# NikNazarov/TorchPIV

Measured on AMD Instinct MI355X. Metric: image-pairs/sec at 4 MP, wind=64 ov=32 2-pass CWS; % HBM roofline, higher is better.
Workload: dtype u32 exact sums + f64 / f32

## Files before the change

### include/torchpiv_hip.h

```cpp
#ifndef TORCHPIV_HIP_H
#define TORCHPIV_HIP_H

#include <stddef.h>
#include <stdint.h>

#ifdef __cplusplus
extern "C" {
#endif

#define TPIV_VERSION 2

enum tpiv_status {
    TPIV_OK = 0,
    TPIV_EINVAL = 1,
    TPIV_EKEY = 2,
    TPIV_EHIP = 3,
    TPIV_ENOMEM = 4,
    TPIV_EUNSUPPORTED = 5
};

enum tpiv_mode {
    TPIV_MODE_DWS = 1,
    TPIV_MODE_CWS = 2,
    TPIV_MODE_CWS_FAST = 3
// ... 115 lines not shown

int tpiv_read_files(const char* const* paths, int n_files, uint8_t* dst, size_t slot_bytes, int n_threads,
                    int64_t* sizes);

typedef struct tpiv_reader tpiv_reader;
tpiv_reader* tpiv_reader_open(const char* const* paths, int64_t n_files, int files_per_batch, uint8_t* const* bufs,
                              int n_bufs, size_t slot_bytes, int n_threads);
int tpiv_reader_next(tpiv_reader* reader, int* n_files, int* buf_index, int64_t* sizes);
int tpiv_reader_release(tpiv_reader* reader);
void tpiv_reader_close(tpiv_reader* reader);


int tpiv_plan_set_timing(tpiv_plan* plan, int enable);
int tpiv_plan_get_timing(tpiv_plan* plan, double* avg_ms, int n_slots, int* n_runs);
int tpiv_plan_exact_fallbacks(tpiv_plan* plan, long long* n_windows);
int tpiv_plan_exact_timing(const tpiv_plan* plan, double* ms4);


int tpiv_debug_pass(int mode, int precision, const uint8_t* a_dev, const uint8_t* b_dev, int batch, int H, int W,
                    int ws, int ov, const double* u2_dev, const double* v2_dev, const double* zero_dev,
                    double* u_dev, double* v_dev, uint8_t* invalid_dev,
                    float* win_dev, float* corr_dev, void* work_dev, size_t work_bytes, void* stream);

int tpiv_debug_iter_compact(int mode, const uint8_t* a_dev, const uint8_t* b_dev, int batch, int H, int W,
                            int ws, int ov, const double* u_raw_dev, const double* v_raw_dev, const uint8_t* mask_dev,
                            double val_ratio, int val_win, int precision,
                            double* u_dev, double* v_dev, uint8_t* invalid_dev, double* du_dev, double* dv_dev,
                            void* work_dev, size_t work_bytes, void* stream);

int tpiv_debug_peaks(const float* maps_dev, int n_maps, int ws, int planar, double val_ratio, int val_win,
                     double* u_dev, double* v_dev, uint8_t* invalid_dev,
                     void* work_dev, size_t work_bytes, void* stream);
// ... 10 lines not shown
```

### torchpiv_amd/_lib.py

```python
from __future__ import annotations

import ctypes as C
import os

_HERE = os.path.dirname(os.path.abspath(__file__))
LIB_PATH = os.environ.get("TPIV_LIB") or os.path.join(_HERE, "libtorchpiv_hip.so")

OK, EINVAL, EKEY, EHIP, ENOMEM, EUNSUPPORTED = 0, 1, 2, 3, 4, 5
MODE_DWS, MODE_CWS, MODE_CWS_FAST = 1, 2, 3
MODES = {"DWS": MODE_DWS, "CWS": MODE_CWS}
ITER_MODES = dict(MODES, CWS_Fast=MODE_CWS_FAST)
PREC_FAST, PREC_REFERENCE, PREC_F64, PREC_EXACT = 0, 1, 2, 3
PRECISIONS = {"fast": PREC_FAST, "reference": PREC_REFERENCE, "f64": PREC_F64, "exact": PREC_EXACT}
PREFILTER_NONE, PREFILTER_MIN, PREFILTER_MEAN = 0, 1, 2
PREFILTERS = {None: PREFILTER_NONE, "min": PREFILTER_MIN, "mean": PREFILTER_MEAN}
ABI_VERSION = 2


class HipError(RuntimeError):
    pass


def _load():
    if not os.path.exists(LIB_PATH):
# ... 19 lines not shown
    "tpiv_coordinates": (C.c_int, [_int, _int, _int, _int, C.POINTER(C.c_double), C.POINTER(C.c_double)]),
    "tpiv_spline_matrix": (C.c_int, [_int, C.POINTER(C.c_double), _int, C.POINTER(C.c_double),
                                     C.POINTER(C.c_double)]),
    "tpiv_pass1": (C.c_int, [_u8p, _u8p, _int, _int, _int, _int, _int, _dbl, _int, _int, _f64p, _f64p, _u8p,
                             _vp, C.c_size_t, _vp]),
    "tpiv_work_bytes": (C.c_size_t, [_int, _int, _int, _int, _int]),
    "tpiv_predict": (C.c_int, [_int, _int, _int, _int, _int, _int, _f64p, _f64p, _f64p, _f64p, _u8p,
                               _f64p, _f64p, _f64p, _f64p, _f64p, _vp]),
    "tpiv_iter": (C.c_int, [_int, _u8p, _u8p, _int, _int, _int, _int, _int, _f64p, _f64p, _f64p, _f64p,
                            _dbl, _int, _int, _f64p, _f64p, _u8p, _f64p, _f64p, _vp, C.c_size_t, _vp]),
    "tpiv_plan_create": (C.c_int, [C.POINTER(C.c_void_p), _int, _int, _int, _int, _int, _int, _dbl, _dbl,
                                   _int, _int, _int]),
    "tpiv_plan_kernel_name": (C.c_char_p, [C.c_void_p, _int, C.c_char_p, _int]),
    "tpiv_plan_exact_fallbacks": (_int, [C.c_void_p, C.POINTER(C.c_longlong)]),
    "tpiv_plan_exact_timing": (_int, [C.c_void_p, C.POINTER(C.c_double)]),
    "tpiv_plan_destroy": (None, [C.c_void_p]),
    "tpiv_plan_n_pass": (C.c_int, [C.c_void_p]),
    "tpiv_plan_pass_geometry": (C.c_int, [C.c_void_p, _int, C.POINTER(C.c_int), C.POINTER(C.c_int),
                                          C.POINTER(C.c_int), C.POINTER(C.c_int)]),
    "tpiv_plan_run": (C.c_int, [C.c_void_p, _u8p, _u8p, _int, _f64p, _f64p, _u8p, _vp]),
    "tpiv_plan_pass_fields": (C.c_int, [C.c_void_p, _int, C.POINTER(C.c_void_p), C.POINTER(C.c_void_p),
                                        C.POINTER(C.c_void_p)]),
    "tpiv_median_test": (C.c_int, [_f64p, _f64p, _u8p, _int, _int, _int, _dbl, _dbl, _int, _u8p, _f64p, _f64p, _vp]),
    "tpiv_plan_set_outlier": (C.c_int, [C.c_void_p, _int, _dbl, _dbl, _int]),
    "tpiv_plan_pass_outliers": (C.c_int, [C.c_void_p, _int, C.POINTER(C.c_void_p)]),
    "tpiv_postval": (C.c_int, [_f64p, _f64p, _u8p, _int, _int, _int, _u8p, _vp, _vp]),
    "tpiv_postval_compact": (C.c_int, [_f64p, _f64p, _u8p, _vp, _int, _int, _int, _vp, _vp, _f64p, _vp, _vp]),
    "tpiv_finish_fields": (C.c_int, [_f64p, _f64p, _int, _int, _int, C.c_double, C.c_double, _f64p, _f64p, _vp]),
    "tpiv_ensemble_moments": (C.c_int, [_f64p, _f64p, _int, C.c_longlong, _f64p, _vp]),
    "tpiv_bmp_unpack": (C.c_int, [_u8p, _vp, _u8p, _int, _int, _int, _u8p, _vp]),
# ... 49 lines not shown
```

### torchpiv_amd/csrc/c_api.cpp

```cpp
#include "../../include/torchpiv_hip.h"

#include <hip/hip_runtime.h>

#include <fcntl.h>
#include <sys/stat.h>
#include <unistd.h>

#include <algorithm>
#include <atomic>
#include <condition_variable>
#include <mutex>
#include <cmath>
#include <cstdio>
#include <cstring>
#include <string>
#include <thread>
#include <vector>

#include "piv_kernels.h"

namespace {

thread_local std::string g_err;
#ifdef TPIV_STAMPS
// ... 173 lines not shown
struct tpiv_plan {
    int H = 0, W = 0, n_pass = 0, mode = 0, max_batch = 0, val_win = 3, device = 0, precision = 0;
    double val_ratio = 1.2;
    std::vector<PassGeo> geo;
    std::vector<double*> u, v;
    std::vector<uint8_t*> val;
    std::vector<double*> Ay, Ax;
    std::vector<double*> Wy32, Ax32;
    std::vector<int*> k0y32, k0x32;
    std::vector<int> KY, KX;
    double *u0 = nullptr, *v0 = nullptr, *T = nullptr;
    uint8_t* pmask = nullptr;
    float* peak_raw = nullptr;
    size_t peak_raw_bytes = 0;
    int last_batch = 0;
    unsigned* exact_count = nullptr;
    int outlier_kind = 0, outlier_min = 3;
    double outlier_threshold = 2.0, outlier_eps = 0.1;
    std::vector<uint8_t*> ostatus;
    double *raw_u = nullptr, *raw_v = nullptr;
    uint8_t* raw_val = nullptr;
    std::vector<void*> allocs;
    bool timing = false;
    std::vector<std::vector<hipEvent_t>> events;
    size_t runs_recorded = 0;

    ~tpiv_plan() {
        for (void* p : allocs) (void)hipFree(p);
        for (auto& r : events)
            for (hipEvent_t e : r) (void)hipEventDestroy(e);
// ... 198 lines not shown
    q.v_c = v_c;
    q.val_c = invalid_c;
    q.T = work;
    q.u0 = u0;
    q.v0 = v0;
    q.u2 = u2;
    q.v2 = v2;
    HIP_TRY(tpiv::launch_predict(q, (hipStream_t)stream));
    return TPIV_OK;
}

static int run_iter(int mode, int precision, const uint8_t* a, const uint8_t* b, int batch, int H, int W, int ws,
                    int ov, const double* u0, const double* v0, const double* u2, const double* v2,
                    double val_ratio, int val_win, double* u, double* v, uint8_t* invalid, double* du,
                    double* dv, float* dbg_win, float* dbg_corr, void* work, size_t work_bytes, void* stream,
                    const uint8_t* pmask = nullptr) {
    if (mode != TPIV_MODE_DWS && mode != TPIV_MODE_CWS && mode != TPIV_MODE_CWS_FAST)
        return fail(TPIV_EKEY, "unknown multipass mode");
    int rc = check_window(H, W, ws, ov, val_win);
    if (rc) return rc;
    if (mode == TPIV_MODE_CWS_FAST && ws < 2) return fail(TPIV_EINVAL, "window too small");
    if (mode != TPIV_MODE_CWS_FAST && !pmask && (!u2 || !v2)) return fail(TPIV_EINVAL, "tpiv_iter: u2 / v2 missing");
    if (!u0 || !v0) return fail(TPIV_EINVAL, "tpiv_iter: u0 / v0 missing");
    if (!valid_precision(precision)) return fail(TPIV_EINVAL, "precision must be TPIV_PREC_FAST, TPIV_PREC_REFERENCE, TPIV_PREC_F64 or TPIV_PREC_EXACT");
    if (batch <= 0) return TPIV_OK;
    tpiv::PassParams p{};
    p.A = a;
    p.B = b;
    p.batch = batch;
    p.H = H;
    p.W = W;
// ... 4 lines not shown
    p.u0 = u0;
    p.v0 = v0;
    p.u2 = u2;
    p.v2 = v2;
    p.pmask = pmask;
    p.u = u;
    p.v = v;
    p.val = invalid;
    p.du = du;
    p.dv = dv;
    p.val_ratio = val_ratio;
    p.val_win = val_win;
    p.dbg_win = dbg_win;
    p.dbg_corr = dbg_corr;
    p.stamps = g_stamps;
    rc = check_work(work, work_bytes,
                    tpiv::peak_raw_bytes(ws, batch, p.n_rows * p.n_cols, TPIV_PREC_FAST, mode == TPIV_MODE_CWS_FAST));
    if (rc) return rc;
    p.peak_raw = static_cast<float*>(work);
    int n_cu;
    rc = n_cu_of_current_device(&n_cu);
    if (rc) return rc;
    HIP_TRY(tpiv::launch_xcorr(p, mode, n_cu, (hipStream_t)stream));
    return TPIV_OK;
}

int tpiv_iter(int mode, const uint8_t* a, const uint8_t* b, int batch, int H, int W, int ws, int ov,
              const double* u0, const double* v0, const double* u2, const double* v2,
              double val_ratio, int val_win, int precision, double* u, double* v, uint8_t* invalid, double* du,
              double* dv, void* work, size_t work_bytes, void* stream) {
// ... 130 lines not shown
            if (t_dense > max_T) max_T = t_dense;
        }
    }
    if (rc == TPIV_OK) {
        size_t raw = 0;
        for (size_t i = 0; i < pl->geo.size(); ++i) {
            const PassGeo& g = pl->geo[i];
            const size_t b = tpiv::peak_raw_bytes(g.ws, max_batch, g.n_rows * g.n_cols,
                                                  i == 0 ? precision : (int)TPIV_PREC_FAST);
            if (b > raw) raw = b;
        }
        pl->peak_raw_bytes = raw;
        if (raw) rc = pl->alloc(&pl->peak_raw, raw / sizeof(float) + 64);
        if (rc == TPIV_OK && precision == TPIV_PREC_EXACT && tpiv::exact_refine_size(pl->geo[0].ws))
            rc = pl->alloc(&pl->exact_count, 4);
    }
    if (rc == TPIV_OK && n_pass > 1) {
        rc = pl->alloc(&pl->u0, max_fine * max_batch);
        if (!rc) rc = pl->alloc(&pl->v0, max_fine * max_batch);
        if (!rc) rc = pl->alloc(&pl->pmask, max_fine * max_batch);
        if (!rc) rc = pl->alloc(&pl->T, max_T * max_batch);
    }
    if (rc) {
        const std::string keep = g_err;
        delete pl;
        g_err = keep;
        return rc;
    }
    *out = pl;
    return TPIV_OK;
// ... 18 lines not shown
    buf[0] = 0;
    if (!plan || pass < 0 || pass >= plan->n_pass) return buf;
    const int mode = pass == 0 ? (int)tpiv::MODE_PASS1 : plan->mode;
    return tpiv::xcorr_kernel_name(plan->geo[pass].ws, mode, plan->precision, buf, len);
}

int tpiv_plan_exact_fallbacks(tpiv_plan* plan, long long* n_windows) {
    if (!plan || !n_windows) return fail(TPIV_EINVAL, "null argument");
    if (!plan->exact_count)
        return fail(TPIV_EINVAL, "not a TPIV_PREC_EXACT plan with an even first-pass window size from 8 to 128");
    if (plan->last_batch <= 0) return fail(TPIV_EINVAL, "the plan has not run yet");
    HIP_TRY(hipDeviceSynchronize());
    unsigned n = 0;
    HIP_TRY(hipMemcpy(&n, plan->exact_count, sizeof(n), hipMemcpyDeviceToHost));
    *n_windows = (long long)n;
    return TPIV_OK;
}

int tpiv_plan_pass_fields(const tpiv_plan* plan, int pass, double** u, double** v, uint8_t** invalid) {
    if (!plan || pass < 0 || pass >= plan->n_pass - 1)
        return fail(TPIV_EINVAL, "only the passes before the last keep their fields in the plan");
    if (u) *u = plan->u[pass];
    if (v) *v = plan->v[pass];
    if (invalid) *invalid = plan->val[pass];
    return TPIV_OK;
}

static int run_banded_predict(tpiv_plan* plan, int p, int batch, const double* u_c, const double* v_c,
                              const uint8_t* val_c, double* u0, double* v0, double* u2, double* v2,
                              hipStream_t st, uint8_t* mask_out = nullptr) {
// ... 161 lines not shown
            if (!rc && plan->exact_count) {
                const size_t off = tpiv::exact_fallback_count_offset(batch, g.n_rows * g.n_cols);
                HIP_TRY(hipMemcpyAsync(plan->exact_count, reinterpret_cast<const char*>(plan->peak_raw) + off,
                                       sizeof(unsigned), hipMemcpyDeviceToDevice, st));
            }
        } else {
            const PassGeo& c = plan->geo[p - 1];
            mark(2 * p - 1, 0);
            rc = run_banded_predict(plan, p, batch, plan->u[p - 1], plan->v[p - 1], plan->val[p - 1], plan->u0,
                                    plan->v0, nullptr, nullptr, st, plan->pmask);
            mark(2 * p - 1, 1);
            mark(2 * p, 0);
            if (!rc)
                rc = run_iter(plan->mode, plan->precision, a, b, batch, plan->H, plan->W, g.ws, g.ov, plan->u0, plan->v0,
                              nullptr, nullptr, plan->val_ratio, plan->val_win, pu, pv, pval, nullptr,
                              nullptr, nullptr, nullptr, plan->peak_raw, plan->peak_raw_bytes, stream, plan->pmask);
            mark(2 * p, 1);
        }
        if (rc) return rc;
        if (test) {
            rc = run_median_test(pu, pv, pval, batch, g.n_rows, g.n_cols, plan->outlier_threshold, plan->outlier_eps,
                                 plan->outlier_min, plan->ostatus[p], p < last ? fu : nullptr, p < last ? fv : nullptr, 1,
                                 p < last ? nullptr : fval, st);
            if (rc) return rc;
        }
    }
    if (plan->timing && plan->runs_recorded < 512) plan->runs_recorded++;
    return TPIV_OK;
}

int tpiv_postval(double* u, double* v, const uint8_t* invalid, int batch, int n_rows, int n_cols, uint8_t* cls,
                 int32_t* counts, void* stream) {
    if (batch < 0 || n_rows < 1 || n_cols < 1) return fail(TPIV_EINVAL, "tpiv_postval: empty grid");
    if ((long long)n_rows * n_cols >= (1LL << 31)) return fail(TPIV_EUNSUPPORTED, "field too large");
    if (batch == 0) return TPIV_OK;
    if (!u || !v || !invalid || !cls || !counts) return fail(TPIV_EINVAL, "tpiv_postval: null pointer");
    tpiv::PostvalParams q{};
    q.u = u;
    q.v = v;
    q.invalid = invalid;
    q.cls = cls;
    q.counts = counts;
    q.batch = batch;
// ... 351 lines not shown
```

### torchpiv_amd/csrc/piv_kernels.h

```cpp
#pragma once
#include <hip/hip_runtime.h>
#include <stdint.h>

namespace tpiv {

enum { MODE_PASS1 = 0, MODE_DWS = 1, MODE_CWS = 2, MODE_CWSF = 3 };

struct PassParams {
    const uint8_t* A;
    const uint8_t* B;
    int batch, H, W;
    int ws, ov, n_rows, n_cols;
    const double* u0;
    const double* v0;
    const double* u2;
    const double* v2;
    const uint8_t* pmask;
    double* u;
    double* v;
    uint8_t* val;
    double* du;
    double* dv;
    double val_ratio;
    int val_win;
// ... 2 lines not shown
    float* dbg_corr;
    unsigned long long* stamps;
    float* peak_raw;
    unsigned* work_ctr;
    int* slow_list;
    unsigned* slow_count;
    int list_mode;
    uint4* cand;
    int* fb_list;
    unsigned* fb_count;
    float exact_band;
    float exact_band_range;
    hipEvent_t* sub_events;
    unsigned groups_magic, ncols_magic;
    int groups_shift, ncols_shift;
};

constexpr double EXACT_ETA = 6.66;
enum { EXACT_FFT_RADIX2 = 0, EXACT_FFT_MIXED = 1, EXACT_FFT_PLAIN = 2 };
inline double exact_gamma_u(int ws, int kind) {
    double lg = 0.0, rt = 1.0;
    for (int n = 1; n < ws; n *= 2) lg += 1.0;
    while ((rt + 1.0) * (rt + 1.0) <= (double)ws) rt += 1.0;
    rt += 1.0;
    const double f1 = kind == EXACT_FFT_PLAIN ? (ws + 3) * rt : (kind == EXACT_FFT_MIXED ? 64.0 : lg * EXACT_ETA);
    const double i1 = kind == EXACT_FFT_PLAIN ? (double)(ws + 3) : f1;
    return 2.0 * (2.0 * f1 + 1.0) + 5.0 + 2.0 * i1;
}
inline float exact_band_coef(int ws, int kind = EXACT_FFT_RADIX2) {
    return (float)(2.0 * exact_gamma_u(ws, kind) * (1.0 + 1.0 / 16) * 5.9604644775390625e-08);
// ... 81 lines not shown
    const double* v;
    const uint8_t* invalid;
    int batch, n_rows, n_cols;
    double threshold, eps;
    int min_neighbours;
    uint8_t* status;
    double* out_u;
    double* out_v;
    int replace;
    uint8_t* invalid_out;
};
hipError_t launch_median_test(const OutlierParams& p, hipStream_t stream);

hipError_t launch_xcorr(const PassParams& p, int mode, int n_cu, hipStream_t stream);
constexpr size_t TILE_CTR_BYTES = 8 * 16 * sizeof(unsigned), TILE_SLOW_HDR_BYTES = 256;
constexpr bool tile_split64(int ws, int mode) { return ws == 64 && mode == MODE_CWS; }
constexpr int tile_occ_c(int ws, int mode) {
    return (ws != 8 && ws != 16 && ws != 32 && ws != 64) ? 0
           : (ws == 16 ? 4 : ((ws == 32 || (ws == 64 && mode != MODE_CWS)) ? 3 : 2));
}
inline int tile_occ(int ws, int mode) { return tile_occ_c(ws, mode); }
#ifdef __HIPCC__
template <int MODE>
__device__ __forceinline__ void pred_half_shift(const PassParams& p, size_t i, double& sx, double& sy) {
    const bool compact = p.pmask != nullptr;
    const double* __restrict__ us = compact ? p.u0 : p.u2;
    const double* __restrict__ vs = compact ? p.v0 : p.v2;
    double u = us[i], v = vs[i];
    if constexpr (MODE == MODE_DWS) {
        const uint8_t* mp = compact ? p.pmask + i : reinterpret_cast<const uint8_t*>(us + i);
        const bool zero = *mp != 0 && compact;
// ... 12 lines not shown
    const float k = compact ? 0.5f : 1.0f;
    vx = (float)us[i] * k;
    vy = (float)vs[i] * k;
}
__device__ __forceinline__ void pred_fallback(const PassParams& p, size_t i, double& u0, double& v0) {
    const bool compact = p.pmask != nullptr;
    const uint8_t* mp = compact ? p.pmask + i : reinterpret_cast<const uint8_t*>(p.u0 + i);
    const bool zero = *mp != 0 && compact;
    u0 = zero ? 0.0 : p.u0[i];
    v0 = zero ? 0.0 : p.v0[i];
}
#endif

const char* xcorr_kernel_name(int ws, int mode, int precision, char* buf, int len);
size_t peak_raw_bytes(int ws, int batch, int n_windows, int precision, bool force_generic = false);
bool exact_refine_size(int ws);
size_t exact_fallback_count_offset(int batch, int n_windows);
hipError_t launch_peaks_from_maps(const PassParams& p, const float* maps, int n_maps, int planar, hipStream_t stream);
hipError_t launch_predict_mfma(const BandedPredictParams& q, hipStream_t stream);
hipError_t launch_predict(const PredictParams& q, hipStream_t stream);

}
```

### torchpiv_amd/csrc/piv_launch.hip

```cpp
#include <hip/hip_runtime.h>
#include <stdint.h>
#include <stdio.h>
#include <stdlib.h>

#include "piv_kernels.h"

namespace tpiv {

hipError_t launch_xcorr_w8(const PassParams& p, int mode, int n_cu, hipStream_t stream);
hipError_t launch_peak_debug_w8(const PassParams& p, const float* maps, int n_maps, hipStream_t stream);
hipError_t launch_xcorr_ws16(const PassParams& p, int mode, int n_cu, hipStream_t stream);
hipError_t launch_xcorr_ws32(const PassParams& p, int mode, int n_cu, hipStream_t stream);
hipError_t launch_xcorr_ws64(const PassParams& p, int mode, int n_cu, hipStream_t stream);
hipError_t launch_xcorr_big128_pass1(const PassParams& p, int n_cu, hipStream_t stream);
hipError_t launch_peak_debug_ws8(const PassParams& p, const float* maps, int n_maps, int planar, hipStream_t stream);
hipError_t launch_peak_debug_ws16(const PassParams& p, const float* maps, int n_maps, int planar, hipStream_t stream);
hipError_t launch_peak_debug_ws32(const PassParams& p, const float* maps, int n_maps, int planar, hipStream_t stream);
hipError_t launch_peak_debug_ws64(const PassParams& p, const float* maps, int n_maps, int planar, hipStream_t stream);
hipError_t launch_peak_debug_ws128(const PassParams& p, const float* maps, int n_maps, hipStream_t stream);
hipError_t launch_xcorr_generic(const PassParams& p, int mode, int n_cu, void* scratch, hipStream_t stream);
int generic_blocks(int ws, long long items, int n_cu, int elem_bytes);
bool generic_ct_usable(int ws);
int generic_ct_register_size(int ws, int mode);
hipError_t launch_xcorr_f64(const PassParams& p, int n_cu, hipStream_t stream);
// ... 156 lines not shown
    if (!tile_size(ws) && ws != 128)
        l.total += (size_t)generic_blocks(ws, (long long)batch * n_windows, 256, 8) * 2 * ws * ws * 2 * 8;
    return l;
}
static bool exact_size(int ws) { return exact_refine_size(ws); }
size_t exact_fallback_count_offset(int batch, int n_windows) { return exact_layout(64, batch, n_windows).count; }

size_t peak_raw_bytes(int ws, int batch, int n_windows, int precision, bool force_generic) {
    if (precision == 3) {
        if (exact_size(ws) && !force_generic) return exact_layout(ws, batch, n_windows).total;
        precision = 1;
    }
    if (tile_size(ws) && !force_generic) {
        if (precision) return peak_bytes(batch, n_windows, 1);
        return work_ctr_offset(batch, n_windows) + WORK_CTR_BYTES +
               (ws == 64 ? TILE_SLOW_HDR_BYTES + (size_t)batch * n_windows * sizeof(int) : 0);
    }
    const int eb = precision ? 8 : 4;
    return peak_bytes(batch, n_windows, precision) +
           (size_t)generic_blocks(ws, (long long)batch * n_windows, 256, eb) * 2 * ws * ws * 2 * eb;
}

static int pass_precision(int precision, int mode, int ws) {
    if (precision == 2) return mode == MODE_PASS1 ? 1 : 0;
    if (precision == 3) return mode == MODE_PASS1 ? (exact_size(ws) ? 3 : 1) : 0;
    return precision;
}

const char* xcorr_kernel_name(int ws, int mode, int precision, char* buf, int len) {
    precision = pass_precision(precision, mode, ws);
    if (precision == 3 && mode == MODE_PASS1) {
        if (ws == 128) snprintf(buf, len, "xcorr_big128_cand_kernel");
        else if (tile_size(ws)) snprintf(buf, len, "xcorr_tile_cand_kernel<%d>", ws);
        else if (generic_ct_usable(ws)) snprintf(buf, len, "xcorr_generic_ct_kernel<0, %d> (cand)", generic_ct_register_size(ws, mode));
        else snprintf(buf, len, "xcorr_generic_kernel<0, float> (cand)");
    } else if (precision && mode == MODE_PASS1) {
        if (ws == 64 || ws == 128) snprintf(buf, len, "xcorr_f64_split_kernel<%d>", ws);
        else if (tile_size(ws)) snprintf(buf, len, "xcorr_f64_tile_kernel<%d>", ws);
        else snprintf(buf, len, "xcorr_generic_kernel<0, double>");
    } else if (ws == 8) {
        snprintf(buf, len, "xcorr_w8_kernel<%d, %s>", mode, (precision && mode != MODE_PASS1) ? "false" : "true");
    } else if (tile_size(ws)) {
// ... 73 lines not shown
            e = launch_xcorr_f64_list(p, n_cu, stream);
        } else {
            q.precision = 1;
            q.cand = nullptr;
            e = launch_xcorr_generic(q, MODE_PASS1, 256, gscratch, stream);
        }
        mark(2);
    } else if (f64) {
        e = (tile_size(p.ws) || p.ws == 128) ? launch_xcorr_f64(p, n_cu, stream) : generic();
    } else if (tile_size(p.ws)) {
        p.work_ctr = reinterpret_cast<unsigned*>(reinterpret_cast<char*>(p.peak_raw) +
                                                 work_ctr_offset(p.batch, p.n_rows * p.n_cols));
        p.list_mode = 0;
        p.slow_list = nullptr;
        p.slow_count = nullptr;
        const bool split = tile_split64(p.ws, mode) && p.precision == 0;
        if (split) {
            p.slow_count = reinterpret_cast<unsigned*>(reinterpret_cast<char*>(p.work_ctr) + WORK_CTR_BYTES);
            p.slow_list = reinterpret_cast<int*>(reinterpret_cast<char*>(p.slow_count) + TILE_SLOW_HDR_BYTES);
        }
        e = hipMemsetAsync(p.work_ctr, 0, WORK_CTR_BYTES + (split ? TILE_SLOW_HDR_BYTES : 0), stream);
        if (e != hipSuccess) return e;
        switch (p.ws) {
            case 8: e = launch_xcorr_w8(p, mode, n_cu, stream); break;
            case 16: e = launch_xcorr_ws16(p, mode, n_cu, stream); break;
            case 32: e = launch_xcorr_ws32(p, mode, n_cu, stream); break;
            default: e = launch_xcorr_ws64(p, mode, n_cu, stream); break;
        }
    } else if (p.ws == 128 && mode == MODE_PASS1) {
        e = launch_xcorr_big128_pass1(p, n_cu, stream);
    } else {
// ... 92 lines not shown
```

### torchpiv_amd/csrc/xcorr_tile.hpp

```cpp
#pragma once
#include <hip/hip_runtime.h>
#include <stdint.h>

#include "fft_inreg.hpp"
#include "piv_kernels.h"

namespace tpiv {

template <int WS, bool PLANAR_ = false>
struct TileGeo {
    static constexpr int WPW = 64 / WS;
    static constexpr int TS = WS > 32 ? 32 : WS;
    static constexpr int PITCH = TS + 1;
    static constexpr int NT = 64 / TS;
    static constexpr int TILE = TS * PITCH;
    static constexpr bool PLANAR = PLANAR_;
    static constexpr int HROWS = WS / 2 + 1;
    static constexpr int HTILE = HROWS * PITCH;
    static constexpr int LDS_FLOATS = NT * TILE * (PLANAR ? 1 : 2);
    static constexpr int MAP_PITCH = WS + 1;
    static constexpr int NDW = WS / 4;
};

template <int CTRL>
// ... 853 lines not shown
            wave_sync();
        }
        sa = 0.f;
        sb = 0.f;
        if constexpr (!FAST) {
#pragma unroll
            for (int k = 0; k < WS; ++k) {
                sa += x[k].x;
                sb += x[k].y;
            }
        }
    }
}

template <int WS>
__device__ __forceinline__ unsigned long long exclusion_row_mask(int m, int ys, int wv) {
    static_assert(WS <= 64, "one 64-bit mask per row");
    const int my_ = m / WS, mx_ = m % WS, KD = WS * WS;
    const int dj = ys - my_;
    unsigned long long ex = 0ull;
    auto span = [&](int lo_, int hi_) TPIV_LAMBDA_INLINE {
        lo_ = lo_ < 0 ? 0 : lo_;
        hi_ = hi_ > WS - 1 ? WS - 1 : hi_;
        if (lo_ > hi_) return 0ull;
        const unsigned long long ones = (hi_ - lo_ + 1) >= 64 ? ~0ull : ((1ull << (hi_ - lo_ + 1)) - 1ull);
        return ones << lo_;
    };
    if (dj >= -wv && dj <= wv) ex |= span(mx_ - wv, mx_ + wv);
    if (dj + 1 >= -wv && dj + 1 <= wv) ex |= span(mx_ - wv + WS, mx_ + wv + WS);
    if (dj - 1 >= -wv && dj - 1 <= wv) ex |= span(mx_ - wv - WS, mx_ + wv - WS);
// ... 318 lines not shown
            if constexpr (MODE == MODE_CWS) {
                pred_half_shift_cws_f32(p, g.fidx, vx, vy);
            } else {
                double sx, sy;
                pred_half_shift<MODE>(p, g.fidx, sx, sy);
                vx = (float)sx;
                vy = (float)sy;
            }
        }
    };

    int item = q_take(q_issue());
    if (item >= hi) return;
    int nitem = q_take(q_issue());
    constexpr bool RECOMPUTE = WS >= 32;
    float vx, vy;
    RawRows<WS, MODE> raw;
    ItemGeom gcur;
    CoopOff<WS> coff;
    if constexpr (MODE == MODE_CWS) coff.init(fresh_lane() % WS, p.W);
    {
        const int l0 = fresh_lane();
        gcur = geom_of(item, l0 / WS);
        shift_of(gcur, vx, vy);
        issue_rows<WS, MODE, FAST>(p, gcur, l0 % WS, vx, vy, raw, coff);
    }

    TPIV_STAMP_DECL
    TPIV_STAMP_START;
    for (int nnitem; item < hi; item = nitem, nitem = nnitem) {
// ... 18 lines not shown
                nnitem = q_take(q_raw);
                issue_rows<WS, MODE, FAST>(p, gnext, r, nvx, nvy, raw, coff);
                vx = nvx;
                vy = nvy;
                if constexpr (!RECOMPUTE) gcur = gnext;
                continue;
            }
        }
        cf x[WS];
        float sa, sb;
        constexpr int NBS = WS >= 32 ? G::WPW : 1;
        int band_s[NBS];
        TPIV_STAMP(0);
        RowSquares sq;
        convert_rows<WS, MODE, RBH, FAST, CAND, ROLE == 1 ? 1 : 0>(p, g, r, lane, vx, vy, raw, x, sa, sb, tile, &sq);
        TPIV_STAMP(1);
        if constexpr (WS >= 64) nnitem = q_take(q_raw);
        if constexpr (WS <= 32) issue_rows<WS, MODE, FAST>(p, gnext, r, nvx, nvy, raw, coff);

        if (p.dbg_win != nullptr && active) {
            int rr = r;
            asm volatile("" : "+v"(rr));
            float* d = p.dbg_win + fidx * 2 * WS * WS + rr * WS;
#pragma unroll
            for (int k = 0; k < WS; ++k) {
                d[k] = x[k].x;
                d[WS * WS + k] = x[k].y;
            }
        }

        bool dead = false;
        float end_scale = 1.0f;
        constexpr bool FASTN = FAST && MODE != MODE_PASS1;
// ... 173 lines not shown
            TPIV_STAMP(8);
            c2r_inreg<WS>(hs, z);
            static_for<0, WS>([&](auto xc) TPIV_LAMBDA_INLINE {
                constexpr int x_ = decltype(xc)::value;
                crow[x_] = (x_ & 1) ? z[FFT_POS<x_ / 2, WS / 2>].y : z[FFT_POS<x_ / 2, WS / 2>].x;
            });
        }
        wave_sync();
        TPIV_STAMP(9);

        auto band_of = [&](int w_) TPIV_LAMBDA_INLINE {
            int b_ = band_s[0];
            static_for<1, NBS>([&](auto wc) TPIV_LAMBDA_INLINE { b_ = w_ == decltype(wc)::value ? band_s[decltype(wc)::value] : b_; });
            return __int_as_float(b_);
        };
        if constexpr (WS > 32) {
            const int lane_p = fresh_lane();
            issue_rows<WS, MODE, FAST>(p, geom_of(nit, lane_p / WS), lane_p % WS, nvx, nvy, raw, coff);
        }
        vx = nvx;
        vy = nvy;
        if constexpr (!RECOMPUTE) gcur = gnext;

        TPIV_STAMP(10);
        if constexpr (RECOMPUTE) {
            const int lane_e = fresh_lane();
            const int w_e = lane_e / WS, r_e = lane_e % WS;
            const int item_e = real_item(item);
            const int pair_e = fast_div(item_e, p.groups_magic, p.groups_shift);
            const int win_raw_e = (item_e - pair_e * groups) * G::WPW + w_e;
            const bool active_e = win_raw_e < N;
// ... 5 lines not shown
            if constexpr (CAND) peak_candidates<WS>(p, crow, tile, w, r, active, dead, fidx, band_of(w));
            else peak_analysis<WS, PLANAR, FASTN>(p, crow, tile, w, r, active, dead, fidx, end_scale);
        }
        wave_sync();
        if constexpr (WS < 64) nnitem = q_take(q_raw);
        TPIV_STAMP(13);
    }
    TPIV_STAMP_FLUSH(p);
}

template <int WS, int MODE, int OCC, bool FAST>
__global__ __launch_bounds__(64, OCC) void xcorr_tile_kernel(PassParams p) {
    xcorr_tile_body<WS, MODE, OCC, FAST, false>(p);
}
template <int WS, int MODE>
__global__ __launch_bounds__(64, 3) void xcorr_tile_fastpath_kernel(PassParams p) {
    xcorr_tile_body<WS, MODE, 3, true, false, 1>(p);
}
template <int WS>
__global__ __launch_bounds__(64, tile_occ_c(WS, MODE_PASS1)) void xcorr_tile_cand_kernel(PassParams p) {
    xcorr_tile_body<WS, MODE_PASS1, tile_occ_c(WS, MODE_PASS1), true, true>(p);
}

template <int WS, bool PLANAR>
__global__ __launch_bounds__(64, 2) void peak_debug_kernel(PassParams p, const float* maps, int n_maps) {
    using G = TileGeo<WS, PLANAR>;
    __shared__ float tile[G::LDS_FLOATS];
    const int lane = threadIdx.x;
    const int w = lane / WS, r = lane % WS;
    const int win_raw = blockIdx.x * G::WPW + w;
    const bool active = win_raw < n_maps;
    const int win = active ? win_raw : n_maps - 1;
// ... 29 lines not shown
    return (unsigned)((blocks + 7) / 8 * 8);
}

template <int WS, int MODE>
static hipError_t launch_tile(const PassParams& p_in, int n_cu, hipStream_t stream) {
    PassParams p = p_in;
    const unsigned blocks = tile_grid<WS>(p, n_cu);
    if (blocks == 0) return hipErrorInvalidValue;
    constexpr int OCC = tile_occ_c(WS, MODE);
    if constexpr (MODE != MODE_PASS1) {
        if (p.precision != 0) {
            hipLaunchKernelGGL((xcorr_tile_kernel<WS, MODE, OCC, false>), dim3(blocks), dim3(64), 0, stream, p);
            return hipGetLastError();
        }
    }
    if constexpr (tile_split64(WS, MODE)) {
        if (p.slow_list != nullptr && p.slow_count != nullptr) {
            hipLaunchKernelGGL((xcorr_tile_fastpath_kernel<WS, MODE>), dim3(blocks), dim3(64), 0, stream, p);
            hipError_t e_ = hipGetLastError();
            if (e_ != hipSuccess) return e_;
            e_ = hipMemsetAsync(p.work_ctr, 0, TILE_CTR_BYTES, stream);
            if (e_ != hipSuccess) return e_;
            PassParams q = p;
            q.list_mode = 1;
            long long blocks2 = (long long)n_cu * 8;
            if (blocks2 > blocks) blocks2 = blocks;
            blocks2 = (blocks2 + 7) / 8 * 8;
            hipLaunchKernelGGL((xcorr_tile_kernel<WS, MODE, OCC, true>), dim3((unsigned)blocks2), dim3(64), 0, stream, q);
            return hipGetLastError();
        }
    }
// ... 25 lines not shown
```

### torchpiv_amd/engine.py

```python
from __future__ import annotations

import ctypes as C

import numpy as np
import torch

from . import _lib
from ._lib import ITER_MODES, MODES, PRECISIONS, check, lib


def _stream() -> int:
    return torch.cuda.current_stream().cuda_stream


def _need_cuda(*tensors):
    for t in tensors:
        if t is not None and not t.is_cuda:
            raise RuntimeError("torchpiv_amd: the HIP path needs tensors on a ROCm device "
                               "(there is no CPU fallback)")


def _frames(a: torch.Tensor, b: torch.Tensor):
    _need_cuda(a, b)
    if a.dtype != torch.uint8 or b.dtype != torch.uint8:
# ... 691 lines not shown

    def kernel_name(self, p):
        buf = C.create_string_buffer(128)
        lib.tpiv_plan_kernel_name(self._h, p, buf, 128)
        return buf.value.decode()

    def exact_capable(self):
        ws = self.geometry[0][0]
        return self.precision == "exact" and 8 <= ws <= 128 and ws % 2 == 0

    def exact_fallbacks(self):
        n = C.c_longlong()
        check(lib.tpiv_plan_exact_fallbacks(self._h, C.byref(n)))
        return n.value

    def exact_timing(self):
        arr = (C.c_double * 4)()
        check(lib.tpiv_plan_exact_timing(self._h, arr))
        return dict(zip(("locate_f32", "refine_exact", "undecided_f64", "finalize"), list(arr)))

    def debug_predict(self, p, u_c, v_c, inv_c):
        B = u_c.shape[0]
        _, _, nr, nc = self.geometry[p]
        outs = [torch.empty(B, nr, nc, dtype=torch.float64, device=self.device) for _ in range(4)]
        with torch.cuda.device(self.device):
            check(lib.tpiv_plan_debug_predict(self._h, p, B, u_c.contiguous().data_ptr(),
                                              v_c.contiguous().data_ptr(), inv_c.contiguous().data_ptr(),
                                              *[o.data_ptr() for o in outs], _stream()))
        return outs

# ... 52 lines not shown
```

Before: 18890.

## Extend fast/slow split tile kernel to 32-pixel windows in CWS passes

Enables the two-launch split (a fast-path kernel followed by a list-driven slow kernel for the remaining items) for ws=32 as well as ws=64 in CWS mode. The ws=32 fast path gets occupancy 4, a late row-issue schedule and an asm register pin on the sample order. The idea is to spend the full-cost kernel only on windows that need it. In exchange it adds an extra launch, a memset and slow-list bookkeeping for the second pass. Debug hooks for forcing a single launch, replaying the last pass and reading slow-item counts are also added.

```diff
diff --git a/include/torchpiv_hip.h b/include/torchpiv_hip.h
--- a/include/torchpiv_hip.h
+++ b/include/torchpiv_hip.h
@@ -153,8 +153,14 @@
 int tpiv_plan_set_timing(tpiv_plan* plan, int enable);
 int tpiv_plan_get_timing(tpiv_plan* plan, double* avg_ms, int n_slots, int* n_runs);
 int tpiv_plan_exact_fallbacks(tpiv_plan* plan, long long* n_windows);
+int tpiv_plan_slow_items(tpiv_plan* plan, int pass, long long* n_items);
 int tpiv_plan_exact_timing(const tpiv_plan* plan, double* ms4);
 
+
+int tpiv_plan_debug_single_launch(tpiv_plan* plan, int on);
+int tpiv_plan_debug_last_pass(tpiv_plan* plan, const uint8_t* a_dev, const uint8_t* b_dev, int batch, const double* u_raw_dev,
+                              const double* v_raw_dev, const uint8_t* mask_dev, double* u_dev, double* v_dev,
+                              uint8_t* invalid_dev, void* stream);
 
 int tpiv_debug_pass(int mode, int precision, const uint8_t* a_dev, const uint8_t* b_dev, int batch, int H, int W,
                     int ws, int ov, const double* u2_dev, const double* v2_dev, const double* zero_dev,
diff --git a/torchpiv_amd/_lib.py b/torchpiv_amd/_lib.py
--- a/torchpiv_amd/_lib.py
+++ b/torchpiv_amd/_lib.py
@@ -57,6 +57,9 @@
     "tpiv_plan_kernel_name": (C.c_char_p, [C.c_void_p, _int, C.c_char_p, _int]),
     "tpiv_plan_exact_fallbacks": (_int, [C.c_void_p, C.POINTER(C.c_longlong)]),
     "tpiv_plan_exact_timing": (_int, [C.c_void_p, C.POINTER(C.c_double)]),
+    "tpiv_plan_slow_items": (_int, [C.c_void_p, _int, C.POINTER(C.c_longlong)]),
+    "tpiv_plan_debug_single_launch": (_int, [C.c_void_p, _int]),
+    "tpiv_plan_debug_last_pass": (_int, [C.c_void_p, _u8p, _u8p, _int, _f64p, _f64p, _u8p, _f64p, _f64p, _u8p, _vp]),
     "tpiv_plan_destroy": (None, [C.c_void_p]),
     "tpiv_plan_n_pass": (C.c_int, [C.c_void_p]),
     "tpiv_plan_pass_geometry": (C.c_int, [C.c_void_p, _int, C.POINTER(C.c_int), C.POINTER(C.c_int),
diff --git a/torchpiv_amd/csrc/c_api.cpp b/torchpiv_amd/csrc/c_api.cpp
--- a/torchpiv_amd/csrc/c_api.cpp
+++ b/torchpiv_amd/csrc/c_api.cpp
@@ -211,6 +211,9 @@
     float* peak_raw = nullptr;
     size_t peak_raw_bytes = 0;
     int last_batch = 0;
+    unsigned* slow_counts = nullptr;
+    std::vector<char> ran_split;
+    bool single_launch = false;
     unsigned* exact_count = nullptr;
     int outlier_kind = 0, outlier_min = 3;
     double outlier_threshold = 2.0, outlier_eps = 0.1;
@@ -439,7 +442,7 @@
                     int ov, const double* u0, const double* v0, const double* u2, const double* v2,
                     double val_ratio, int val_win, double* u, double* v, uint8_t* invalid, double* du,
                     double* dv, float* dbg_win, float* dbg_corr, void* work, size_t work_bytes, void* stream,
-                    const uint8_t* pmask = nullptr) {
+                    const uint8_t* pmask = nullptr, int single_launch = 0) {
     if (mode != TPIV_MODE_DWS && mode != TPIV_MODE_CWS && mode != TPIV_MODE_CWS_FAST)
         return fail(TPIV_EKEY, "unknown multipass mode");
     int rc = check_window(H, W, ws, ov, val_win);
@@ -474,6 +477,7 @@
     p.dbg_win = dbg_win;
     p.dbg_corr = dbg_corr;
     p.stamps = g_stamps;
+    p.single_launch = single_launch;
     rc = check_work(work, work_bytes,
                     tpiv::peak_raw_bytes(ws, batch, p.n_rows * p.n_cols, TPIV_PREC_FAST, mode == TPIV_MODE_CWS_FAST));
     if (rc) return rc;
@@ -634,6 +638,10 @@
         if (raw) rc = pl->alloc(&pl->peak_raw, raw / sizeof(float) + 64);
         if (rc == TPIV_OK && precision == TPIV_PREC_EXACT && tpiv::exact_refine_size(pl->geo[0].ws))
             rc = pl->alloc(&pl->exact_count, 4);
+        pl->ran_split.assign(pl->geo.size(), 0);
+        bool keeps_count = false;
+        for (size_t i = 1; i + 1 < pl->geo.size(); ++i) keeps_count |= tpiv::xcorr_pass_splits(pl->geo[i].ws, mode, precision);
+        if (rc == TPIV_OK && keeps_count) rc = pl->alloc(&pl->slow_counts, pl->geo.size());
     }
     if (rc == TPIV_OK && n_pass > 1) {
         rc = pl->alloc(&pl->u0, max_fine * max_batch);
@@ -682,6 +690,29 @@
     unsigned n = 0;
     HIP_TRY(hipMemcpy(&n, plan->exact_count, sizeof(n), hipMemcpyDeviceToHost));
     *n_windows = (long long)n;
+    return TPIV_OK;
+}
+
+int tpiv_plan_slow_items(tpiv_plan* plan, int pass, long long* n_items) {
+    if (!plan || !n_items || pass < 0 || pass >= plan->n_pass) return fail(TPIV_EINVAL, "bad plan / pass index");
+    if (plan->last_batch <= 0) return fail(TPIV_EINVAL, "the plan has not run yet");
+    HIP_TRY(hipDeviceSynchronize());
+    *n_items = 0;
+    if (!plan->ran_split[pass]) return TPIV_OK;
+    const PassGeo& g = plan->geo[pass];
+    const void* src = pass == plan->n_pass - 1
+                          ? static_cast<const void*>(reinterpret_cast<const char*>(plan->peak_raw) +
+                                                     tpiv::tile_slow_count_offset(plan->last_batch, g.n_rows * g.n_cols))
+                          : static_cast<const void*>(plan->slow_counts + pass);
+    unsigned n = 0;
+    HIP_TRY(hipMemcpy(&n, src, sizeof(n), hipMemcpyDeviceToHost));
+    *n_items = (long long)n;
+    return TPIV_OK;
+}
+
+int tpiv_plan_debug_single_launch(tpiv_plan* plan, int on) {
+    if (!plan) return fail(TPIV_EINVAL, "null plan");
+    plan->single_launch = on != 0;
     return TPIV_OK;
 }
 
@@ -873,8 +904,15 @@
             if (!rc)
                 rc = run_iter(plan->mode, plan->precision, a, b, batch, plan->H, plan->W, g.ws, g.ov, plan->u0, plan->v0,
                               nullptr, nullptr, plan->val_ratio, plan->val_win, pu, pv, pval, nullptr,
-                              nullptr, nullptr, nullptr, plan->peak_raw, plan->peak_raw_bytes, stream, plan->pmask);
+                              nullptr, nullptr, nullptr, plan->peak_raw, plan->peak_raw_bytes, stream, plan->pmask,
+                              plan->single_launch ? 1 : 0);
             mark(2 * p, 1);
+            plan->ran_split[p] = !plan->single_launch && tpiv::xcorr_pass_splits(g.ws, plan->mode, plan->precision);
+            if (!rc && plan->ran_split[p] && p < last) {
+                const size_t off = tpiv::tile_slow_count_offset(batch, g.n_rows * g.n_cols);
+                HIP_TRY(hipMemcpyAsync(plan->slow_counts + p, reinterpret_cast<const char*>(plan->peak_raw) + off,
+                                       sizeof(unsigned), hipMemcpyDeviceToDevice, st));
+            }
         }
         if (rc) return rc;
         if (test) {
@@ -886,6 +924,31 @@
     }
     if (plan->timing && plan->runs_recorded < 512) plan->runs_recorded++;
     return TPIV_OK;
+}
+
+int tpiv_plan_debug_last_pass(tpiv_plan* plan, const uint8_t* a, const uint8_t* b, int batch, const double* u_raw,
+                              const double* v_raw, const uint8_t* mask, double* u, double* v, uint8_t* invalid, void* stream) {
+    if (!plan) return fail(TPIV_EINVAL, "null plan");
+    const int last = plan->n_pass - 1;
+    if (last < 1) return fail(TPIV_EINVAL, "tpiv_plan_debug_last_pass: the plan has one pass only");
+    if (batch < 1 || batch > plan->max_batch) return fail(TPIV_EINVAL, "batch exceeds the plan's max_batch");
+    if (!u_raw || !v_raw || !mask) return fail(TPIV_EINVAL, "tpiv_plan_debug_last_pass: predictor missing");
+    int dev = 0;
+    HIP_TRY(hipGetDevice(&dev));
+    if (dev != plan->device) return fail(TPIV_EINVAL, "plan was created on another device");
+    const PassGeo& g = plan->geo[last];
+    const bool test = plan->outlier_kind != 0;
+    uint8_t* const pval = test ? plan->raw_val : invalid;
+    plan->last_batch = batch;
+    int rc = run_iter(plan->mode, plan->precision, a, b, batch, plan->H, plan->W, g.ws, g.ov, u_raw, v_raw, nullptr, nullptr,
+                      plan->val_ratio, plan->val_win, u, v, pval, nullptr, nullptr, nullptr, nullptr, plan->peak_raw,
+                      plan->peak_raw_bytes, stream, mask, plan->single_launch ? 1 : 0);
+    if (rc) return rc;
+    plan->ran_split[last] = !plan->single_launch && tpiv::xcorr_pass_splits(g.ws, plan->mode, plan->precision);
+    if (test)
+        rc = run_median_test(u, v, pval, batch, g.n_rows, g.n_cols, plan->outlier_threshold, plan->outlier_eps,
+                             plan->outlier_min, plan->ostatus[last], nullptr, nullptr, 1, invalid, (hipStream_t)stream);
+    return rc;
 }
 
 int tpiv_postval(double* u, double* v, const uint8_t* invalid, int batch, int n_rows, int n_cols, uint8_t* cls,
diff --git a/torchpiv_amd/csrc/piv_kernels.h b/torchpiv_amd/csrc/piv_kernels.h
--- a/torchpiv_amd/csrc/piv_kernels.h
+++ b/torchpiv_amd/csrc/piv_kernels.h
@@ -40,6 +40,7 @@
     hipEvent_t* sub_events;
     unsigned groups_magic, ncols_magic;
     int groups_shift, ncols_shift;
+    int single_launch;
 };
 
 constexpr double EXACT_ETA = 6.66;
@@ -151,7 +152,8 @@
 
 hipError_t launch_xcorr(const PassParams& p, int mode, int n_cu, hipStream_t stream);
 constexpr size_t TILE_CTR_BYTES = 8 * 16 * sizeof(unsigned), TILE_SLOW_HDR_BYTES = 256;
-constexpr bool tile_split64(int ws, int mode) { return ws == 64 && mode == MODE_CWS; }
+constexpr bool tile_split(int ws, int mode) { return (ws == 64 || ws == 32) && mode == MODE_CWS; }
+constexpr int tile_fastpath_occ_c(int ws) { return ws == 32 ? 4 : 3; }
 constexpr int tile_occ_c(int ws, int mode) {
     return (ws != 8 && ws != 16 && ws != 32 && ws != 64) ? 0
            : (ws == 16 ? 4 : ((ws == 32 || (ws == 64 && mode != MODE_CWS)) ? 3 : 2));
@@ -194,6 +196,8 @@
 
 const char* xcorr_kernel_name(int ws, int mode, int precision, char* buf, int len);
 size_t peak_raw_bytes(int ws, int batch, int n_windows, int precision, bool force_generic = false);
+bool xcorr_pass_splits(int ws, int mode, int precision);
+size_t tile_slow_count_offset(int batch, int n_windows);
 bool exact_refine_size(int ws);
 size_t exact_fallback_count_offset(int batch, int n_windows);
 hipError_t launch_peaks_from_maps(const PassParams& p, const float* maps, int n_maps, int planar, hipStream_t stream);
diff --git a/torchpiv_amd/csrc/piv_launch.hip b/torchpiv_amd/csrc/piv_launch.hip
--- a/torchpiv_amd/csrc/piv_launch.hip
+++ b/torchpiv_amd/csrc/piv_launch.hip
@@ -194,7 +194,7 @@
     if (tile_size(ws) && !force_generic) {
         if (precision) return peak_bytes(batch, n_windows, 1);
         return work_ctr_offset(batch, n_windows) + WORK_CTR_BYTES +
-               (ws == 64 ? TILE_SLOW_HDR_BYTES + (size_t)batch * n_windows * sizeof(int) : 0);
+               (tile_split(ws, MODE_CWS) ? TILE_SLOW_HDR_BYTES + (size_t)batch * n_windows * sizeof(int) : 0);
     }
     const int eb = precision ? 8 : 4;
     return peak_bytes(batch, n_windows, precision) +
@@ -206,6 +206,11 @@
     if (precision == 3) return mode == MODE_PASS1 ? (exact_size(ws) ? 3 : 1) : 0;
     return precision;
 }
+
+bool xcorr_pass_splits(int ws, int mode, int precision) {
+    return mode != MODE_PASS1 && tile_split(ws, mode) && pass_precision(precision, mode, ws) == 0;
+}
+size_t tile_slow_count_offset(int batch, int n_windows) { return work_ctr_offset(batch, n_windows) + WORK_CTR_BYTES; }
 
 const char* xcorr_kernel_name(int ws, int mode, int precision, char* buf, int len) {
     precision = pass_precision(precision, mode, ws);
@@ -309,7 +314,7 @@
         p.list_mode = 0;
         p.slow_list = nullptr;
         p.slow_count = nullptr;
-        const bool split = tile_split64(p.ws, mode) && p.precision == 0;
+        const bool split = tile_split(p.ws, mode) && p.precision == 0 && !p.single_launch;
         if (split) {
             p.slow_count = reinterpret_cast<unsigned*>(reinterpret_cast<char*>(p.work_ctr) + WORK_CTR_BYTES);
             p.slow_list = reinterpret_cast<int*>(reinterpret_cast<char*>(p.slow_count) + TILE_SLOW_HDR_BYTES);
diff --git a/torchpiv_amd/csrc/xcorr_tile.hpp b/torchpiv_amd/csrc/xcorr_tile.hpp
--- a/torchpiv_amd/csrc/xcorr_tile.hpp
+++ b/torchpiv_amd/csrc/xcorr_tile.hpp
@@ -891,6 +891,13 @@
 }
 
 template <int WS>
+__device__ __forceinline__ void pin_sample_order(cf (&x)[WS]) {
+    static_assert(WS == 32, "written out for 32 samples");
+    asm volatile("" : "+v"(x[0].y), "+v"(x[1].y), "+v"(x[2].y), "+v"(x[3].y), "+v"(x[4].y), "+v"(x[5].y), "+v"(x[6].y), "+v"(x[7].y), "+v"(x[8].y), "+v"(x[9].y), "+v"(x[10].y), "+v"(x[11].y), "+v"(x[12].y), "+v"(x[13].y), "+v"(x[14].y), "+v"(x[15].y), "+v"(x[16].y), "+v"(x[17].y), "+v"(x[18].y), "+v"(x[19].y), "+v"(x[20].y), "+v"(x[21].y), "+v"(x[22].y), "+v"(x[23].y), "+v"(x[24].y), "+v"(x[25].y), "+v"(x[26].y), "+v"(x[27].y), "+v"(x[28].y), "+v"(x[29].y), "+v"(x[30].y), "+v"(x[31].y));
+    asm volatile("" : "+v"(x[0].x), "+v"(x[1].x), "+v"(x[2].x), "+v"(x[3].x), "+v"(x[4].x), "+v"(x[5].x), "+v"(x[6].x), "+v"(x[7].x), "+v"(x[8].x), "+v"(x[9].x), "+v"(x[10].x), "+v"(x[11].x), "+v"(x[12].x), "+v"(x[13].x), "+v"(x[14].x), "+v"(x[15].x), "+v"(x[16].x), "+v"(x[17].x), "+v"(x[18].x), "+v"(x[19].x), "+v"(x[20].x), "+v"(x[21].x), "+v"(x[22].x), "+v"(x[23].x), "+v"(x[24].x), "+v"(x[25].x), "+v"(x[26].x), "+v"(x[27].x), "+v"(x[28].x), "+v"(x[29].x), "+v"(x[30].x), "+v"(x[31].x));
+}
+
+template <int WS>
 __device__ __forceinline__ unsigned long long exclusion_row_mask(int m, int ys, int wv) {
     static_assert(WS <= 64, "one 64-bit mask per row");
     const int my_ = m / WS, mx_ = m % WS, KD = WS * WS;
@@ -1239,6 +1246,7 @@
     if (item >= hi) return;
     int nitem = q_take(q_issue());
     constexpr bool RECOMPUTE = WS >= 32;
+    constexpr bool LATE_ISSUE = WS > 32 || (ROLE == 1 && OCC >= 4);
     float vx, vy;
     RawRows<WS, MODE> raw;
     ItemGeom gcur;
@@ -1287,9 +1295,12 @@
         TPIV_STAMP(0);
         RowSquares sq;
         convert_rows<WS, MODE, RBH, FAST, CAND, ROLE == 1 ? 1 : 0>(p, g, r, lane, vx, vy, raw, x, sa, sb, tile, &sq);
+        if constexpr (ROLE == 1 && WS == 32) {
+            pin_sample_order(x);
+        }
         TPIV_STAMP(1);
         if constexpr (WS >= 64) nnitem = q_take(q_raw);
-        if constexpr (WS <= 32) issue_rows<WS, MODE, FAST>(p, gnext, r, nvx, nvy, raw, coff);
+        if constexpr (!LATE_ISSUE) issue_rows<WS, MODE, FAST>(p, gnext, r, nvx, nvy, raw, coff);
 
         if (p.dbg_win != nullptr && active) {
             int rr = r;
@@ -1493,7 +1504,7 @@
             static_for<1, NBS>([&](auto wc) TPIV_LAMBDA_INLINE { b_ = w_ == decltype(wc)::value ? band_s[decltype(wc)::value] : b_; });
             return __int_as_float(b_);
         };
-        if constexpr (WS > 32) {
+        if constexpr (LATE_ISSUE) {
             const int lane_p = fresh_lane();
             issue_rows<WS, MODE, FAST>(p, geom_of(nit, lane_p / WS), lane_p % WS, nvx, nvy, raw, coff);
         }
@@ -1529,8 +1540,8 @@
     xcorr_tile_body<WS, MODE, OCC, FAST, false>(p);
 }
 template <int WS, int MODE>
-__global__ __launch_bounds__(64, 3) void xcorr_tile_fastpath_kernel(PassParams p) {
-    xcorr_tile_body<WS, MODE, 3, true, false, 1>(p);
+__global__ __launch_bounds__(64, tile_fastpath_occ_c(WS)) void xcorr_tile_fastpath_kernel(PassParams p) {
+    xcorr_tile_body<WS, MODE, tile_fastpath_occ_c(WS), true, false, 1>(p);
 }
 template <int WS>
 __global__ __launch_bounds__(64, tile_occ_c(WS, MODE_PASS1)) void xcorr_tile_cand_kernel(PassParams p) {
@@ -1590,7 +1601,7 @@
             return hipGetLastError();
         }
     }
-    if constexpr (tile_split64(WS, MODE)) {
+    if constexpr (tile_split(WS, MODE)) {
         if (p.slow_list != nullptr && p.slow_count != nullptr) {
             hipLaunchKernelGGL((xcorr_tile_fastpath_kernel<WS, MODE>), dim3(blocks), dim3(64), 0, stream, p);
             hipError_t e_ = hipGetLastError();
diff --git a/torchpiv_amd/engine.py b/torchpiv_amd/engine.py
--- a/torchpiv_amd/engine.py
+++ b/torchpiv_amd/engine.py
@@ -729,6 +729,31 @@
         check(lib.tpiv_plan_exact_fallbacks(self._h, C.byref(n)))
         return n.value
 
+    def slow_items(self, p):
+        n = C.c_longlong()
+        check(lib.tpiv_plan_slow_items(self._h, p, C.byref(n)))
+        return n.value
+
+    def debug_single_launch(self, on: bool):
+        check(lib.tpiv_plan_debug_single_launch(self._h, 1 if on else 0))
+
+    def debug_last_pass(self, a, b, u_raw, v_raw, mask, out=None):
+        a, b = _frames(a, b)
+        B = a.shape[0]
+        nr, nc = self.out_shape
+        _need_cuda(u_raw, v_raw, mask)
+        for t, dt in ((u_raw, torch.float64), (v_raw, torch.float64), (mask, torch.uint8)):
+            if t.dtype != dt or tuple(t.shape) != (B, nr, nc) or not t.is_contiguous():
+                raise ValueError(f"predictor fields must be contiguous [{B}, {nr}, {nc}] float64 / uint8")
+        if out is None:
+            u = torch.empty(B, nr, nc, dtype=torch.float64, device=a.device)
+            out = (u, torch.empty_like(u), torch.empty(B, nr, nc, dtype=torch.uint8, device=a.device))
+        u, v, inv = out
+        with torch.cuda.device(self.device):
+            check(lib.tpiv_plan_debug_last_pass(self._h, a.data_ptr(), b.data_ptr(), B, u_raw.data_ptr(), v_raw.data_ptr(),
+                                                mask.data_ptr(), u.data_ptr(), v.data_ptr(), inv.data_ptr(), _stream()))
+        return u, v, inv
+
     def exact_timing(self):
         arr = (C.c_double * 4)()
         check(lib.tpiv_plan_exact_timing(self._h, arr))
```

Result: no change. 18990 (median of 6 runs) (+0.5%).
